# MilchRatchet/Luminary

Measured on AMD Instinct MI355X. Metric: Mrays/s at 1920x1080, 8 bounces, higher is better.
Workload: dtype f32

## Files before the change

include/lum_core.h:

```cpp
#ifndef LUM_CORE_H
#define LUM_CORE_H

#include <stdint.h>

#ifdef __cplusplus
extern "C" {
#endif

typedef struct LumContext LumContext;

typedef struct LumDeviceSceneView {
  uint32_t num_meshes;
  uint32_t num_instances;
  uint32_t num_materials;
  uint32_t num_lights;
  const uint32_t* mesh_tri_offset;
  const float* vertices;
  const uint32_t* tri_tex;
  const uint32_t* instance_mesh_ids;
  const float* instance_transforms;
  const uint16_t* materials;
  const uint8_t* light_tree_root;
  const uint8_t* light_tree_nodes;
  const uint32_t* light_tri_handles;
// ... 204 lines not shown
int lumc_frame_assemble(LumContext* ctx, uint32_t frame_pixels, int root, void* stream, float** d_frame_out);
int lumc_frame_assemble_all(LumContext** ctxs, int n, uint32_t frame_pixels, int root, float** d_frame_root);
int lumc_frame_gather(LumContext* ctx, uint32_t width, uint32_t height, int root, void* stream, float** d_frame_out);
int lumc_frame_gather_all(LumContext** ctxs, int n, uint32_t width, uint32_t height, int root, float** d_frame_root);
int lumc_frame_download(LumContext* ctx, uint32_t frame_pixels, float* first_moment, float* second_moment);
uint32_t lumc_frame_plane_stride(const LumContext* ctx);
int lumc_use_assembled_frame(LumContext* ctx, int on);
int lumc_accumulators_from_frame(LumContext* dst, LumContext* src);
int lumc_comm_count(const LumContext* ctx);
int lumc_device_name(int ordinal, char* out, size_t size);

int lumc_set_ray_sorting(LumContext* ctx, int mode);
int lumc_get_ray_sorting(const LumContext* ctx);

enum { LUMC_FLAVOUR_EXACT = 0, LUMC_FLAVOUR_FAST = 1 };
int lumc_set_flavour(LumContext* ctx, int flavour);
int lumc_get_flavour(const LumContext* ctx);
int lumc_set_ambient_reuse(LumContext* ctx, int mode);
int lumc_get_ambient_reuse(const LumContext* ctx);
int lumc_set_single_level(LumContext* ctx, int mode);
int lumc_get_single_level(const LumContext* ctx);
int lumc_set_plain_form(LumContext* ctx, int mode);
int lumc_get_plain_form(const LumContext* ctx);
int lumc_set_fused_resolve(LumContext* ctx, int on);
int lumc_set_sobol_table(LumContext* ctx, int on);
double lumc_bvh_build_seconds(const LumContext* ctx);
int lumc_bvh_meshes_by_builder(const LumContext* ctx, uint32_t out[2]);
int lumc_bvh_stats(LumContext* ctx, uint64_t out[4]);
uint32_t lumc_scene_view_sizeof(void);
int lumc_host_bvh_probe(const float* boxes, uint32_t count, uint32_t max_leaf, uint64_t out[6], double inner_area[3]);
uint32_t lumc_leaf_max_triangles(void);
typedef struct LumMeshRefitStats {
  uint64_t refits, rebuilds;
  uint32_t last_refits, last_rebuilds;
  double max_cost_growth;
  double seconds;
  double seconds_upload, seconds_refit, seconds_rebuild, seconds_assemble;
  double seconds_hash, seconds_download, seconds_lights;
} LumMeshRefitStats;
int lumc_set_mesh_refit(LumContext* ctx, uint32_t mode, float max_cost_growth);
int lumc_mesh_refit_stats(const LumContext* ctx, LumMeshRefitStats* out);
int lumc_bvh_refit_probe(const float* built_boxes, const float* refit_boxes, uint32_t count, uint32_t refit_count, int builder, int on_gpu, uint64_t sizes[3],
                         void* built_nodes, void* refit_nodes, void* host_refit_nodes, uint32_t* prims, double cost[3], uint64_t* valid);
int lumc_scene_tree_probe(const LumDeviceSceneView* scene, uint64_t sizes[4], void* nodes, void* tris, void* leaves, void* rows, uint32_t* mesh_root, float bounds[6]);
typedef struct LumInstanceUpdateStats {
  uint64_t device_updates, fallbacks, relayouts;
// ... 98 lines not shown
```

luminary_amd/core.py:

```python
import ctypes as C

import numpy as np

from . import DeviceSceneView, _lib

DIRTY_CONSTANTS, DIRTY_MATERIALS, DIRTY_INSTANCES, DIRTY_LIGHTS, DIRTY_MESHES, DIRTY_TEXTURES, DIRTY_PARTICLES, DIRTY_ALL = 1, 2, 4, 8, 16, 32, 64, 127
DIRTY_MESH_POSITIONS = 128
DIRTY_INSTANCE_TRANSFORMS = 256
DIRTY_MESH_SKIN = 512
DIRTY_LIGHT_POSITIONS = 1024
DIRTY_MESH_SHUTTER = 2048
BVH_BUILDERS = {"sah": 0, "lbvh": 1, "ploc": 2, "sah_gpu": 3}
CNT_TRACE, CNT_SHADOW, CNT_LIGHT_BVH, CNT_VERTICES, CNT_NODES, CNT_TRIS, CNT_NODES_SHADOW, CNT_TRIS_SHADOW, CNT_NODES_LIGHT, CNT_TRIS_LIGHT, CNT_NODES_LDS, CNT_NODES_LDS_SHADOW, CNT_AMBIENT_DEFERRED, CNT_AMBIENT_FALLBACK = range(14)
CNT_COUNT = 16
KERNELS = ("generate", "trace", "shade", "shadow", "accumulate", "light_query", "resolve", "output", "sky", "sort", "volume")


class CoreError(RuntimeError):
    pass


class OutputParams(C.Structure):
    _fields_ = [("src_width", C.c_uint32), ("src_height", C.c_uint32), ("dst_width", C.c_uint32), ("dst_height", C.c_uint32),
                ("inv_sample_count", C.c_float), ("exposure", C.c_float), ("tonemap", C.c_uint32), ("filter", C.c_uint32), ("dithering", C.c_uint32),
# ... 375 lines not shown

    @property
    def ambient_reuse(self):
        fn = self._lib.lumc_get_ambient_reuse
        fn.restype = C.c_int
        return bool(fn(self._ctx))

    def set_single_level(self, mode):
        self._call("lumc_set_single_level", C.c_int(mode))

    def get_single_level(self):
        fn = self._lib.lumc_get_single_level
        fn.restype = C.c_int
        return int(fn(self._ctx))

    def set_plain_form(self, mode):
        self._call("lumc_set_plain_form", C.c_int(mode))

    def get_plain_form(self):
        fn = self._lib.lumc_get_plain_form
        fn.restype = C.c_int
        return int(fn(self._ctx))

    def set_physical_camera(self, camera):
        self._call("lumc_set_physical_camera", C.byref(camera) if camera is not None else C.c_void_p(0))

    def camera_rays(self, pixels, first_sample, samples):
        px = np.ascontiguousarray(pixels, dtype=np.uint32)
        n = px.size * samples
        o = np.zeros((n, 3), dtype=np.float32)
        d = np.zeros((n, 3), dtype=np.float32)
        w = np.zeros(n, dtype=np.float32)
        self._call("lumc_camera_rays", px.ctypes.data_as(C.c_void_p), C.c_uint32(px.size), C.c_uint32(first_sample), C.c_uint32(samples),
                   o.ctypes.data_as(C.c_void_p), d.ctypes.data_as(C.c_void_p), w.ctypes.data_as(C.c_void_p))
        return o, d, w

    def pixel_query(self, x, y, sample_id=0):
        out = (C.c_uint32 * 6)()
        self._call("lumc_pixel_query", C.c_uint32(x), C.c_uint32(y), C.c_uint32(sample_id), out)
        a = np.array(list(out), dtype=np.uint32)
        return int(a[0]), int(a[1]), float(a[2:3].view(np.float32)[0]), a[3:6].view(np.float32).copy()

    def set_flavour(self, name):
        self._call("lumc_set_flavour", C.c_int({"exact": 0, "fast": 1}[name]))

    def _call(self, name, *args):
# ... 89 lines not shown
    def accumulators(self):
        fm = np.zeros(3 * self.num_pixels, dtype=np.float32)
        sm = np.zeros(self.num_pixels, dtype=np.float32)
        self._call("lumc_download_accumulators", fm.ctypes.data_as(C.c_void_p), sm.ctypes.data_as(C.c_void_p))
        return fm.reshape(3, -1), sm

    def counters(self):
        out = (C.c_uint64 * CNT_COUNT)()
        self._call("lumc_counters", out)
        return [int(x) for x in out]

    def query_counters(self):
        c = self.counters()
        c[CNT_SHADOW] += c[CNT_AMBIENT_DEFERRED] - c[CNT_AMBIENT_FALLBACK]
        return c

    def reset_counters(self):
        self._call("lumc_reset_counters")

    def set_profiling(self, on):
        self._call("lumc_set_profiling", C.c_int(1 if on else 0))

    def kernel_times(self):
        ms = (C.c_double * len(KERNELS))()
        n = (C.c_uint32 * len(KERNELS))()
        self._call("lumc_kernel_times", ms, n)
        return {k: (float(ms[i]), int(n[i])) for i, k in enumerate(KERNELS)}

    def adaptive_begin(self, max_rate, avg_rate, update_interval, exposure=0.0, tone=None):
        p = AdaptiveParams()
        p.max_sampling_rate, p.avg_sampling_rate, p.update_interval, p.exposure = max_rate, avg_rate, update_interval, exposure
        if tone is not None:
            p.tone = tone
        self._call("lumc_adaptive_begin", C.byref(p))

    def adaptive_render(self, executions, stream=0):
        self._call("lumc_adaptive_render", C.c_uint32(executions), C.c_void_p(stream))

    def adaptive_info(self):
        info = AdaptiveInfo()
        self._call("lumc_adaptive_info", C.byref(info))
        return {"stage_id": int(info.stage_id), "executions": [int(x) for x in info.executions], "num_blocks": int(info.num_blocks),
                "blocks": (int(info.blocks_x), int(info.blocks_y)), "tasks_per_execution": int(info.tasks_per_execution),
                "variance_total": float(info.variance_total), "build_pending": bool(info.build_pending)}

    @staticmethod
    def adaptive_info_of(ctx):
# ... 296 lines not shown
```

luminary_amd/csrc/device/wavefront_table.h:

```cpp
#pragma once

#include <hip/hip_runtime.h>

#include "dev_scene.h"

namespace lum {

inline bool single_level_scene(const DeviceScene& sc) { return sc.tlas_num_nodes == 1u && sc.tlas_num_leaves == 2u; }

inline bool plain_scene(const DeviceScene& sc) {
  return (sc.traits & kTraitsPlain) == kTraitsPlain && sc.num_lights <= (uint32_t) LUM_LDS_LIGHTS && !sc.ocean_active &&
         (sc.sky_mode == kSkyConstantColor || sc.sky_mode == kSkyHdri);
}

struct WavefrontKernels {
  const char* flavour;
  uint32_t trace_block;
  int (*set_ray_kernel_lds)(size_t bytes);
  int (*init_sampler_seeds)();
  void (*sobol_table)(hipStream_t s, uint2* table, uint32_t first_sample, uint32_t count, uint32_t stride, uint32_t dims);
  void (*generate)(uint32_t grid, hipStream_t s, const DeviceScene& sc, const PassParams& pp, const PathQueue& q, float4* results, uint32_t* count, const DeviceLens& lens,
                   int cam);
  void (*generate_adaptive)(uint32_t grid, hipStream_t s, const DeviceScene& sc, const AdaptiveView& a, const AdaptivePass& pass, const PathQueue& q, float4* results,
                            uint32_t* count, const DeviceLens& lens, int cam);
// ... 35 lines not shown
  void (*trace_rays)(uint32_t grid, size_t lds, hipStream_t s, const DeviceScene& sc, uint32_t n, const float* origins, const float* dirs, const uint32_t* ignore, uint32_t* out,
                     uint32_t* cursor, uint64_t* counters, uint32_t lds_nodes, bool single_level);
  void (*camera_rays)(uint32_t grid, hipStream_t s, const DeviceScene& sc, const DeviceLens& lens, int cam, const uint32_t* pixels, uint32_t n, uint32_t first_sample,
                      uint32_t samples, float* origin, float* dir, float* weight);
  void (*guide)(uint32_t grid, hipStream_t s, const DeviceScene& sc, const PathQueue& in, const uint32_t* ctrl, float* planes, uint32_t n);
  void (*guide_normalise)(uint32_t grid, hipStream_t s, float* planes, uint32_t n, uint32_t samples);
  void (*denoise_prepare)(uint32_t grid, hipStream_t s, const AdaptiveView& a, const DenoiseArgs& p, const float* fm, const float* sm, const float* image, const float* guides,
                          float4* rec_a, uint4* rec_b);
  void (*denoise_atrous)(hipStream_t s, const DenoiseArgs& p, const float4* a_in, const uint4* rec_b, float4* a_out, bool lds);
  void (*denoise_finish)(uint32_t grid, hipStream_t s, const DenoiseArgs& p, const float4* rec_a, const float* guides, float* image);
  void (*light_query_probe)(hipStream_t s, const DeviceScene& sc, uint32_t n, const float* origins, const float* dirs, const uint32_t* self, const float* randoms, uint32_t* out_ids,
                            uint32_t* out_num_hits);
};
struct WavefrontProbes {
  void (*light_sample_probe)(hipStream_t s, const DeviceScene& sc, uint32_t n_vertices, uint32_t samples, uint32_t first_sample, uint32_t form, const uint32_t* vertices,
                             uint32_t* out);
};
constexpr uint32_t kLightSampleProbeVertexWords = 20, kLightSampleProbeWords = 154;

const WavefrontKernels* wavefront_kernels_exact();
const WavefrontKernels* wavefront_kernels_fast();
const WavefrontProbes* wavefront_probes_exact();
const WavefrontProbes* wavefront_probes_fast();

}
```

luminary_amd/csrc/device/wavefront_table_impl.h:

```cpp
#pragma once

#include "dev_adaptive.h"
#include "dev_denoise.h"
#include "wavefront_table.h"

LUM_NS_BEGIN
namespace table {

typedef void (*TraceKernel)(DeviceScene, PathQueue, const uint32_t*, uint32_t*, uint64_t*, uint32_t);
typedef void (*ShadowKernel)(DeviceScene, ShadowQueue, const uint32_t*, uint32_t*, uint64_t*, uint32_t);
typedef void (*TraceRaysKernel)(DeviceScene, uint32_t, const float*, const float*, const uint32_t*, uint32_t*, uint32_t*, uint64_t*, uint32_t);
static TraceKernel trace_kernel(bool single) { return single ? k_trace<true> : static_cast<TraceKernel>(k_trace); }
static ShadowKernel shadow_kernel(bool single) { return single ? k_shadow_rays<true> : static_cast<ShadowKernel>(k_shadow_rays); }
static TraceRaysKernel trace_rays_kernel(bool single) { return single ? k_trace_rays<true> : static_cast<TraceRaysKernel>(k_trace_rays); }

static int set_ray_kernel_lds(size_t bytes) {
  hipError_t e = hipSuccess;
  for (int single = 0; single < 2 && e == hipSuccess; single++) {
    e = hipFuncSetAttribute((const void*) trace_kernel(single != 0), hipFuncAttributeMaxDynamicSharedMemorySize, (int) bytes);
    if (e == hipSuccess) e = hipFuncSetAttribute((const void*) shadow_kernel(single != 0), hipFuncAttributeMaxDynamicSharedMemorySize, (int) bytes);
    if (e == hipSuccess) e = hipFuncSetAttribute((const void*) trace_rays_kernel(single != 0), hipFuncAttributeMaxDynamicSharedMemorySize, (int) bytes);
  }
  if (e == hipSuccess) e = hipFuncSetAttribute((const void*) k_trace_particles, hipFuncAttributeMaxDynamicSharedMemorySize, (int) bytes);
  return (int) e;
}
static int init_sampler_seeds() { return upload_sampler_seeds(); }
static void sobol_table(hipStream_t s, uint2* table, uint32_t first_sample, uint32_t count, uint32_t stride, uint32_t dims) {
  hipLaunchKernelGGL(k_sobol_table, dim3((dims * stride + 255u) / 256u), dim3(256), 0, s, table, first_sample, count, stride, dims);
}
static void generate(uint32_t grid, hipStream_t s, const DeviceScene& sc, const PassParams& pp, const PathQueue& q, float4* results, uint32_t* count, const DeviceLens& lens,
                     int cam) {
  auto* k = cam == kCamPhysical ? k_generate<kCamPhysical> : cam == kCamPhysicalReflections ? k_generate<kCamPhysicalReflections> : k_generate<kCamThinLens>;
  hipLaunchKernelGGL(k, dim3(grid), dim3(kBlock), 0, s, sc, pp, q, results, count, lens);
}
static void generate_adaptive(uint32_t grid, hipStream_t s, const DeviceScene& sc, const AdaptiveView& a, const AdaptivePass& pass, const PathQueue& q, float4* results,
                              uint32_t* count, const DeviceLens& lens, int cam) {
  auto* k = cam == kCamPhysical ? k_generate_adaptive<kCamPhysical> : cam == kCamPhysicalReflections ? k_generate_adaptive<kCamPhysicalReflections>
                                                                                                     : k_generate_adaptive<kCamThinLens>;
  hipLaunchKernelGGL(k, dim3(grid), dim3(kBlock), 0, s, sc, a, pass, q, results, count, lens);
}
static void camera_rays(uint32_t grid, hipStream_t s, const DeviceScene& sc, const DeviceLens& lens, int cam, const uint32_t* pixels, uint32_t n, uint32_t first_sample,
                        uint32_t samples, float* origin, float* dir, float* weight) {
  auto* k = cam == kCamPhysical ? k_camera_rays<kCamPhysical> : cam == kCamPhysicalReflections ? k_camera_rays<kCamPhysicalReflections> : k_camera_rays<kCamThinLens>;
  hipLaunchKernelGGL(k, dim3(grid), dim3(kBlock), 0, s, sc, lens, pixels, n, first_sample, samples, origin, dir, weight);
}
static void trace(uint32_t grid, size_t lds, hipStream_t s, const DeviceScene& sc, const PathQueue& q, const uint32_t* order, uint32_t* ctrl, uint64_t* counters,
// ... 158 lines not shown
extern "C" int lumc_debug_vis_stats_fast(uint64_t out[8], int reset) {
  if (hipMemcpyFromSymbol(out, HIP_SYMBOL(g_vis_stat), sizeof(uint64_t) * 8) != hipSuccess) return 1;
  if (reset) { const uint64_t zero[8] = {0}; if (hipMemcpyToSymbol(HIP_SYMBOL(g_vis_stat), zero, sizeof(zero)) != hipSuccess) return 1; }
  return 0;
}
extern "C" int lumc_debug_shade_times_fast(uint64_t out[16], int reset) {
  if (hipMemcpyFromSymbol(out, HIP_SYMBOL(g_shade_time), sizeof(uint64_t) * 16) != hipSuccess) return 1;
  if (reset) { const uint64_t zero[16] = {0}; if (hipMemcpyToSymbol(HIP_SYMBOL(g_shade_time), zero, sizeof(zero)) != hipSuccess) return 1; }
  return 0;
}
#else
extern "C" int lumc_debug_phase_stats(uint64_t out[16], int reset) {
  if (hipMemcpyFromSymbol(out, HIP_SYMBOL(g_phase), sizeof(uint64_t) * 16) != hipSuccess) return 1;
  if (reset) { const uint64_t zero[16] = {0}; if (hipMemcpyToSymbol(HIP_SYMBOL(g_phase), zero, sizeof(zero)) != hipSuccess) return 1; }
  return 0;
}
#endif
#endif

namespace lum {
#if LUM_FAST
const WavefrontKernels* wavefront_kernels_fast() { return &fast::table::kTable; }
const WavefrontProbes* wavefront_probes_fast() { return &fast::table::kProbes; }
#else
const WavefrontKernels* wavefront_kernels_exact() { return &exact::table::kTable; }
const WavefrontProbes* wavefront_probes_exact() { return &exact::table::kProbes; }
#endif
}
```

luminary_amd/csrc/host/context.h:

```cpp
#pragma once

#include <hip/hip_runtime.h>

#include <cstdio>
#include <map>
#include <memory>
#include <string>
#include <vector>

#include "../../../include/lum_core.h"
#include "../device/dev_scene.h"
#include "../device/wavefront_table.h"
#include "bvh_build.h"
#include "bvh_refit.h"
#include "device_buffer.h"
#include "instance_update.h"
#include "light_refit.h"
#include "mesh_deform.h"
#include "mesh_shutter.h"
#include "scene_arrays.h"
#include "work_layout.h"

using namespace lum;

// ... 40 lines not shown
  DeviceBuffer<uint32_t> d_skin_flags;
  LumMeshSkinStats skin_stats{};
  LumMeshMorphStats morph_stats{};
  std::map<uint32_t, MeshShutter> mesh_shutter;
  DeviceBuffer<uint32_t> d_shutter_flags;
  LumShutterStats shutter_stats{};
  LightRefit light_refit;
  Bvh4 light_bvh;
  float light_refit_max_cost_growth = 0.0f;
  bool light_refit_needs_rebuild = false;
  bool lights_refitted = false;
  LumLightRefitStats light_refit_stats{};
  std::vector<uint32_t> sky_lut_key;
  DeviceBuffer<float> d_bridge_lut;
  std::vector<float> bridge_lut_host;
  DeviceBuffer<float4> d_sky_lut[2];
  DeviceScene scene{};
  bool has_scene = false;
  uint64_t bvh_stats[4] = {0, 0, 0, 0};
  int ambient_reuse = -1;
  int single_level = -1;
  int plain_form = -1;
  bool first_leaf_identity = false;
  uint32_t shade_grid_rounds = 2;
  int fused_resolve = 1;
  struct Fused : FusedBuffers {
    DeviceBuffer<char> block;
    bool records_stale = false;
    uint32_t refused_capacity = 0;
  } fused;
  DeviceBuffer<uint2> d_sobol;
  int sobol_table = 1;
  int fused_ended = 1;
  int fused_ended_default = 1;
  int bvh_builder = 3;
  double bvh_build_seconds = 0.0;
  uint32_t bvh_meshes_by_builder[2] = {0, 0};
  uint32_t lds_nodes = 0;
  uint32_t trace_blocks = 256;
  DeviceBuffer<uint16_t> d_luts[4];
  DeviceBuffer<uint32_t> d_pixels;
  uint32_t num_pixels = 0;
  uint64_t pixels_hash = 0;
  DeviceBuffer<float> d_first_moment, d_second_moment;
  struct Work : WorkBuffers { DeviceBuffer<char> block; } work;
  uint32_t particle_lds_nodes = 0;
// ... 62 lines not shown
};

#define HIP_TRY(ctx, expr)                                                                                          \
  do {                                                                                                              \
    const hipError_t e__ = (expr);                                                                                  \
    if (e__ != hipSuccess) {                                                                                        \
      (ctx)->error = std::string(#expr) + " failed: " + hipGetErrorString(e__);                                     \
      return 1;                                                                                                     \
    }                                                                                                               \
  } while (0)

#pragma GCC visibility push(hidden)

constexpr uint32_t kLaunchBlock = 256;
inline uint32_t grid_for(uint32_t n) {
  const uint32_t blocks = (n + kLaunchBlock - 1) / kLaunchBlock;
  return blocks < 1 ? 1 : (blocks > 2048 ? 2048 : blocks);
}

inline bool single_level_allowed(const LumContext* ctx) {
  return ctx->single_level != 0 && (ctx->wf != wavefront_kernels_fast() || ctx->first_leaf_identity);
}

inline uint32_t grid_persistent(const LumContext* ctx, uint32_t n) {
  const uint32_t tb = ctx->wf->trace_block;
  const uint32_t blocks = (n + tb - 1) / tb;
  return blocks < 1 ? 1 : (blocks > ctx->trace_blocks ? ctx->trace_blocks : blocks);
}

struct Launch {
  LumContext* ctx;
  hipStream_t stream;
  int kernel;
  size_t idx = (size_t) -1;
  Launch(LumContext* c, hipStream_t s, int k) : ctx(c), stream(s), kernel(k) {
    if (!ctx->profiling) return;
    LumContext::Stamp st;
    st.kernel = k;
    if (hipEventCreate(&st.a) != hipSuccess || hipEventCreate(&st.b) != hipSuccess) return;
    (void) hipEventRecord(st.a, stream);
    ctx->stamps.push_back(st);
    idx = ctx->stamps.size() - 1;
  }
  ~Launch() {
    if (idx != (size_t) -1) (void) hipEventRecord(ctx->stamps[idx].b, stream);
    if (ctx->sync_debug) {
// ... 17 lines not shown
```

luminary_amd/csrc/host/core.hip:

```cpp
#include <hip/hip_runtime.h>

#include <algorithm>
#include <cmath>
#include <cstdio>
#include <cstdlib>
#include <cstring>
#include <string>
#include <vector>

#include "../../../include/lum_core.h"
#include "../device/kernels_shared.h"
#include <hipcub/hipcub.hpp>
#include "context.h"
#include "tiles.h"

static_assert(kLaunchBlock == (uint32_t) kBlock, "grid_for (context.h) counts the kernels' workgroups");

namespace {

void free_work(LumContext* ctx) {
  ctx->work = LumContext::Work{};
  ctx->fused = LumContext::Fused{};
  free_sort(ctx);
  ctx->d_sobol.reset();
// ... 50 lines not shown

inline uint32_t shade_grid(const LumContext* ctx, uint32_t n) {
  const uint32_t blocks = (n + kBlock - 1) / kBlock;
  const uint32_t resident = ctx->trace_blocks * 3u;
  const uint32_t rounds = ctx->shade_grid_rounds;
  const uint32_t cap = resident * (rounds ? rounds : 1u);
  return blocks < 1 ? 1 : std::min(blocks, cap);
}

int resolve_stamps(LumContext* ctx) {
  for (auto& st : ctx->stamps) {
    float ms = 0.0f;
    if (hipEventSynchronize(st.b) == hipSuccess && hipEventElapsedTime(&ms, st.a, st.b) == hipSuccess) {
      ctx->kernel_ms[st.kernel] += ms;
      ctx->kernel_launches[st.kernel]++;
    }
    (void) hipEventDestroy(st.a);
    (void) hipEventDestroy(st.b);
  }
  ctx->stamps.clear();
  return 0;
}

}

extern "C" {

int lumc_context_create(int device_ordinal, LumContext** out) {
  if (!out) return 1;
  *out = nullptr;
  LumContext* ctx = new LumContext();
  ctx->device = device_ordinal;
  if (const char* b = getenv("LUM_BVH_BUILDER")) ctx->bvh_builder = (std::strcmp(b, "lbvh") == 0) ? 1 : (std::strcmp(b, "ploc") == 0) ? 2 : (std::strcmp(b, "sah") == 0 || std::strcmp(b, "host") == 0) ? 0 : 3;
  if (const char* e = getenv("LUM_SORT")) ctx->sort.mode = atoi(e);
  if (const char* e = getenv("LUM_SYNC_DEBUG")) ctx->sync_debug = atoi(e) != 0;
  if (const char* e = getenv("LUM_SORT_KEY")) ctx->sort.key = atoi(e);
  if (const char* e = getenv("LUM_AMBIENT_REUSE")) ctx->ambient_reuse = atoi(e) != 0 ? 1 : 0;
  if (const char* e = getenv("LUM_SINGLE_LEVEL")) ctx->single_level = atoi(e) != 0 ? 1 : 0;
  if (const char* e = getenv("LUM_PLAIN_FORM")) ctx->plain_form = atoi(e) != 0 ? 1 : 0;
  if (const char* e = getenv("LUM_FUSED_RESOLVE")) ctx->fused_resolve = atoi(e) != 0 ? 1 : 0;
  if (const char* e = getenv("LUM_SHADE_GRID")) ctx->shade_grid_rounds = (uint32_t) atoi(e);
  if (const char* e = getenv("LUM_SOBOL_TABLE_RT")) ctx->sobol_table = atoi(e) != 0 ? 1 : 0;
  if (const char* e = getenv("LUM_FUSED_ENDED")) ctx->fused_ended = ctx->fused_ended_default = atoi(e) != 0 ? 1 : 0;
  if (const char* e = getenv("LUM_DENOISE_LDS")) ctx->denoise_lds = atoi(e) != 0 ? 1 : 0;
  if (const char* f = getenv("LUM_FLAVOUR")) ctx->wf = (std::strcmp(f, "exact") == 0) ? wavefront_kernels_exact() : wavefront_kernels_fast();
  *out = ctx;
  int count = 0;
  HIP_TRY(ctx, hipGetDeviceCount(&count));
  if (device_ordinal < 0 || device_ordinal >= count) { ctx->error = "no such HIP device"; return 1; }
  HIP_TRY(ctx, hipSetDevice(device_ordinal));
  HIP_TRY(ctx, (hipError_t) wavefront_kernels_exact()->init_sampler_seeds());
  HIP_TRY(ctx, (hipError_t) wavefront_kernels_fast()->init_sampler_seeds());
  HIP_TRY(ctx, (hipError_t) exact::upload_sampler_seeds());
  HIP_TRY(ctx, (hipError_t) scene_device_init());
  HIP_TRY(ctx, ctx->d_ctrl.resize(kCtlStride * kCtrlRows));
  HIP_TRY(ctx, hipMemset(ctx->d_ctrl.get(), 0, sizeof(uint32_t) * kCtlStride * kCtrlRows));
  HIP_TRY(ctx, ctx->d_counters.resize(LUMC_CNT_COUNT));
  HIP_TRY(ctx, hipMemset(ctx->d_counters.get(), 0, sizeof(uint64_t) * LUMC_CNT_COUNT));
  return 0;
}

void lumc_context_destroy(LumContext* ctx) {
  if (!ctx) return;
  (void) hipSetDevice(ctx->device);
  (void) hipDeviceSynchronize();
  resolve_stamps(ctx);
  free_exchange(ctx);
  delete ctx;
}

const char* lumc_last_error(const LumContext* ctx) { return ctx ? ctx->error.c_str() : "null context"; }
uint32_t lumc_scene_view_sizeof(void) { return (uint32_t) sizeof(LumDeviceSceneView); }

uint64_t pixel_list_hash(const uint32_t* pixels, uint32_t n) {
  uint64_t h = 1469598103934665603ull;
  for (uint32_t i = 0; i < n; i++) { h ^= pixels ? pixels[i] : i; h *= 1099511628211ull; }
  return h;
}

int lumc_set_pixels(LumContext* ctx, const uint32_t* pixels, uint32_t num_pixels) {
  if (!ctx || !ctx->has_scene) { if (ctx) ctx->error = "lumc_set_pixels: no scene"; return 1; }
  HIP_TRY(ctx, hipSetDevice(ctx->device));
  if (!pixels) num_pixels = ctx->scene.width * ctx->scene.height;
  ctx->adaptive = LumContext::Adaptive();
  ctx->d_pixels.reset(); ctx->d_first_moment.reset(); ctx->d_second_moment.reset();
  ctx->num_pixels = num_pixels;
  ctx->pixels_hash = pixel_list_hash(pixels, num_pixels);
  if (num_pixels == 0) return 0;
  HIP_TRY(ctx, ctx->d_pixels.assign(pixels, num_pixels));
// ... 47 lines not shown
  if (sc.particles_active) trace_particles(ctx, stream, ctx->work.queue[0], ctx->d_ctrl.get(), N);
  if (sc.ocean_active) {
    Launch l(ctx, stream, LUMC_KERNEL_TRACE);
    wf.trace_ocean(grid_for(N), stream, sc, ctx->work.queue[0], (const uint32_t*) ctx->d_ctrl.get());
  }
}

static void debug_pass(LumContext* ctx, hipStream_t stream, const DeviceScene& sc, uint32_t N) {
  const WavefrontKernels& wf = *ctx->wf;
  first_hits(ctx, stream, sc, N);
  if (render_volumes(sc)) {
    Launch l(ctx, stream, LUMC_KERNEL_VOLUME);
    wf.volume_events(grid_for(N), stream, sc, ctx->work.queue[0], ctx->work.volume, ctx->work.results, ctx->d_ctrl.get(), 0u);
  }
  if (sc.sky_aerial_perspective && sc.sky_mode != kSkyConstantColor) {
    Launch l(ctx, stream, LUMC_KERNEL_SKY);
    wf.sky_inscattering(grid_for(N), stream, sc, ctx->work.queue[0], ctx->work.results, (const uint32_t*) ctx->d_ctrl.get(), 0u);
  }
  Launch l(ctx, stream, LUMC_KERNEL_SHADE);
  wf.shade_debug(grid_for(N), stream, sc, ctx->work.queue[0], ctx->work.results, (const uint32_t*) ctx->d_ctrl.get());
}

enum ResolveScheme { kResolvePlain, kResolveReuse, kResolveFused };

struct DepthBuffers {
  PathQueue& cur;
  PathQueue& next;
  PathQueue& prev;
  NeeQueue& nee;
  NeeQueue& nee_before;
  uint32_t* ctrl;
  const FusedResolve* fused_records;
  uint32_t* ended;
  uint32_t depth, depth_const;
  bool last;
};

static DepthBuffers depth_buffers(LumContext* ctx, ResolveScheme scheme, uint32_t depth, uint32_t max_depth) {
  const bool fused = scheme == kResolveFused;
  const int cur = fused ? (int) (depth % 3u) : (int) (depth & 1u);
  const int next_q = fused ? (cur + 1) % 3 : (cur ^ 1), prev_q = fused ? (cur + 2) % 3 : (cur ^ 1);
  const bool second_set = fused && (depth & 1u);
  const uint32_t depth_const = (depth == max_depth && depth > 0) ? depth - 1 : depth;
  return DepthBuffers{ctx->work.queue[cur], ctx->work.queue[next_q], ctx->work.queue[prev_q], second_set ? ctx->fused.nee : ctx->work.nee, second_set ? ctx->work.nee : ctx->fused.nee,
                      ctx->d_ctrl.get() + kCtlStride * depth, fused ? ctx->fused.records + depth % 6u : nullptr, fused ? ctx->fused.ended[depth & 1u] : nullptr, depth, depth_const,
                      depth == max_depth};
}

static int closest_hits(LumContext* ctx, hipStream_t stream, const DeviceScene& sc, ResolveScheme scheme, const DepthBuffers& d, uint32_t N) {
  const WavefrontKernels& wf = *ctx->wf;
  const uint32_t* order = nullptr;
  if (ctx->sort.mode >= 1 && d.depth >= 1 && sort_closest_rays(ctx, stream, d.cur, d.ctrl, N, &order)) return 1;
  {
    Launch l(ctx, stream, LUMC_KERNEL_TRACE);
    wf.trace(grid_persistent(ctx, N), ray_kernel_lds(ctx), stream, sc, d.cur, order, d.ctrl, ctx->d_counters.get(), ctx->lds_nodes, single_level_allowed(ctx));
  }
  if (scheme == kResolveReuse && d.depth > 0) {
    uint32_t* prev = d.ctrl - kCtlStride;
    {
      Launch l(ctx, stream, LUMC_KERNEL_RESOLVE);
      wf.resolve_reuse(grid_for(N), stream, sc, d.prev, d.cur, d.nee, ctx->work.shadow, ctx->work.results, prev, ctx->d_counters.get());
    }
    {
      Launch l(ctx, stream, LUMC_KERNEL_SHADOW);
      wf.shadow_rays(ctx->trace_blocks, ray_kernel_lds(ctx), stream, sc, ctx->work.shadow, nullptr, prev + kCtlVolumeShift, ctx->d_counters.get(), ctx->lds_nodes, single_level_allowed(ctx));
    }
    Launch l(ctx, stream, LUMC_KERNEL_RESOLVE);
    wf.resolve_listed(std::min<uint32_t>(grid_for(N), 1024u), stream, sc, d.prev, d.nee, ctx->work.shadow, ctx->work.results, (const uint32_t*) prev);
  }
  return 0;
}

static void media_passes(LumContext* ctx, hipStream_t stream, const DeviceScene& sc, const DepthBuffers& d, uint32_t N) {
  const WavefrontKernels& wf = *ctx->wf;
  if (sc.particles_active) trace_particles(ctx, stream, d.cur, d.ctrl, N);
  if (sc.ocean_active) {
    Launch l(ctx, stream, LUMC_KERNEL_TRACE);
    wf.trace_ocean(grid_for(N), stream, sc, d.cur, (const uint32_t*) d.ctrl);
  }
// ... 37 lines not shown
      wf.shadow_rays(ctx->trace_blocks, ray_kernel_lds(ctx), stream, sc, ctx->fused.fallback, nullptr, d.ctrl + kCtlVolumeShift, ctx->d_counters.get(), ctx->lds_nodes, single_level_allowed(ctx));
    }
    Launch l(ctx, stream, LUMC_KERNEL_RESOLVE);
    wf.resolve_listed(std::min<uint32_t>(grid_for(N), 1024u), stream, sc, d.prev, d.nee_before, ctx->fused.fallback, ctx->work.results, (const uint32_t*) d.ctrl);
  }
}

static void feature_shading(LumContext* ctx, hipStream_t stream, const DeviceScene& sc, const DepthBuffers& d, uint32_t N) {
  const WavefrontKernels& wf = *ctx->wf;
  if (sc.particles_active) {
    Launch l(ctx, stream, LUMC_KERNEL_SHADE);
    wf.particle_shade(grid_for(N), stream, sc, d.cur, d.next, d.nee, ctx->work.shadow, d.ctrl, d.depth_const);
  }
  if (sc.ocean_active) {
    Launch l(ctx, stream, LUMC_KERNEL_SHADE);
    wf.ocean_shade(grid_for(N), stream, sc, d.cur, d.next, d.nee, ctx->work.shadow, d.ctrl, d.depth_const);
  }
  if (sc.sky_mode == kSkyDefault) {
    Launch l(ctx, stream, LUMC_KERNEL_SKY);
    wf.sky(grid_for(N), stream, sc, d.cur, ctx->work.shadow, ctx->work.results, (const uint32_t*) d.ctrl, d.depth_const);
  }
}

static int visibility_and_resolve(LumContext* ctx, hipStream_t stream, const DeviceScene& sc, ResolveScheme scheme, const DepthBuffers& d, uint32_t N) {
  const WavefrontKernels& wf = *ctx->wf;
  {
    Launch l(ctx, stream, LUMC_KERNEL_LIGHT_QUERY);
    wf.light_query(std::min<uint32_t>(grid_for(N), ctx->trace_blocks * 4u), stream, sc, d.cur, d.nee, ctx->work.shadow, d.ctrl, d.depth_const, ctx->d_counters.get());
  }
  const uint32_t* shadow_order = nullptr;
  if (ctx->sort.mode == 2) {
    shadow_order = sort_rays(ctx, stream, ctx->work.shadow.origin_dist, ctx->work.shadow.dir_out, d.ctrl + kCtlShadowItems,
                             (sc.ocean_active ? kSurfaceShadowKindsWater : 4u) * (ctx->work.shadow.capacity < N ? ctx->work.shadow.capacity : N));
    if (!shadow_order) { ctx->error = "ray sorting failed"; return 1; }
  }
  {
    Launch l(ctx, stream, LUMC_KERNEL_SHADOW);
    wf.shadow_rays(grid_persistent(ctx, N), ray_kernel_lds(ctx), stream, sc, ctx->work.shadow, shadow_order, d.ctrl, ctx->d_counters.get(), ctx->lds_nodes, single_level_allowed(ctx));
  }
  if (d.last || scheme == kResolvePlain) {
    Launch l(ctx, stream, LUMC_KERNEL_RESOLVE);
    wf.resolve(grid_for(N), stream, sc, d.cur, d.nee, ctx->work.shadow, ctx->work.results, (const uint32_t*) d.ctrl);
  }
  else if (scheme == kResolveFused) {
    if (!ctx->fused_ended) {
      Launch l(ctx, stream, LUMC_KERNEL_RESOLVE);
      wf.resolve_ended(std::min<uint32_t>(grid_for(N), 4096u), stream, sc, d.cur, d.nee, ctx->work.shadow, ctx->work.results, (const uint32_t*) d.ctrl, d.ended);
    }
  }
  return 0;
}

static void volume_bounce(LumContext* ctx, hipStream_t stream, const DeviceScene& sc, const DepthBuffers& d, uint32_t N) {
  if (render_volumes(sc) && !d.last) {
    Launch l(ctx, stream, LUMC_KERNEL_VOLUME);
    ctx->wf->volume_bounce(grid_for(N), stream, sc, d.cur, d.next, ctx->work.volume, d.ctrl, d.depth_const);
  }
}

static int wavefront_depths(LumContext* ctx, hipStream_t stream, uint32_t N, uint32_t first_sample = 0, uint32_t sample_count = 0) {
  DeviceScene sc = ctx->scene;
  const uint32_t max_depth = sc.max_ray_depth;
  prepare_sobol_table(ctx, stream, sc, first_sample, sample_count);
  if (sc.shading_mode != 0u) { debug_pass(ctx, stream, sc, N); return 0; }
  ResolveScheme scheme = ambient_reuse_active(ctx) ? kResolveReuse : kResolvePlain;
  if (scheme == kResolveReuse && ctx->wf->fused_resolve && ctx->fused_resolve != 0 && ctx->wf == wavefront_kernels_fast() && max_depth > 0) {
    if (ensure_fused(ctx, stream) == 0) scheme = kResolveFused;
    else {
      (void) hipGetLastError();
      ctx->error.clear();
    }
  }
  for (uint32_t depth = 0; depth <= max_depth; depth++) {
    const DepthBuffers d = depth_buffers(ctx, scheme, depth, max_depth);
    if (closest_hits(ctx, stream, sc, scheme, d, N)) return 1;
    media_passes(ctx, stream, sc, d, N);
    shade_depth(ctx, stream, sc, scheme, d, N);
    feature_shading(ctx, stream, sc, d, N);
    if (visibility_and_resolve(ctx, stream, sc, scheme, d, N)) return 1;
    volume_bounce(ctx, stream, sc, d, N);
  }
  return 0;
}

int lumc_render(LumContext* ctx, uint32_t first_sample, uint32_t num_samples, uint32_t samples_per_pass, float* d_fm, float* d_sm, void* stream_) {
  if (!ctx || !ctx->has_scene) { if (ctx) ctx->error = "lumc_render: no scene"; return 1; }
  if (ctx->num_pixels == 0) return 0;
  hipStream_t stream = (hipStream_t) stream_;
  HIP_TRY(ctx, hipSetDevice(ctx->device));
  if (!d_fm) { d_fm = ctx->d_first_moment.get(); d_sm = ctx->d_second_moment.get(); }
  if (samples_per_pass == 0) samples_per_pass = 1;
  if (first_sample >= kMaxGlobalSamples) return 0;
  if (first_sample + (uint64_t) num_samples > kMaxGlobalSamples) num_samples = kMaxGlobalSamples - first_sample;
  const uint32_t P = ctx->num_pixels;
  const uint64_t want = (uint64_t) P * samples_per_pass;
  if (want > 0x7FFFFFFFull) { ctx->error = "pass too large"; return 1; }
  if (ensure_work(ctx, (uint32_t) want)) return 1;
  const DeviceScene& sc = ctx->scene;
  const uint32_t max_depth = sc.max_ray_depth;

  for (uint32_t done = 0; done < num_samples; done += samples_per_pass) {
// ... 857 lines not shown
  return 0;
}
int lumc_set_ambient_reuse(LumContext* ctx, int mode) {
  if (!ctx || mode < -1 || mode > 1) { if (ctx) ctx->error = "lumc_set_ambient_reuse: -1 (by flavour), 0 (off) or 1 (on)"; return 1; }
  ctx->ambient_reuse = mode;
  return 0;
}
int lumc_get_ambient_reuse(const LumContext* ctx) { return (ctx && ambient_reuse_active(ctx)) ? 1 : 0; }

int lumc_set_single_level(LumContext* ctx, int mode) {
  if (!ctx || mode < -1 || mode > 1) { if (ctx) ctx->error = "lumc_set_single_level: -1 (auto), 0 (never) or 1 (when the scene is eligible)"; return 1; }
  ctx->single_level = mode;
  return 0;
}
int lumc_get_single_level(const LumContext* ctx) { return (ctx && ctx->has_scene && single_level_allowed(ctx) && single_level_scene(ctx->scene)) ? 1 : 0; }

int lumc_set_plain_form(LumContext* ctx, int mode) {
  if (!ctx || mode < -1 || mode > 1) { if (ctx) ctx->error = "lumc_set_plain_form: -1 (auto), 0 (never) or 1 (when the scene is eligible)"; return 1; }
  ctx->plain_form = mode;
  return 0;
}

int lumc_get_plain_form(const LumContext* ctx) { return (ctx && ctx->has_scene && ctx->plain_form != 0 && plain_scene(ctx->scene)) ? 1 : 0; }
int lumc_get_flavour(const LumContext* ctx) { return (ctx && ctx->wf == wavefront_kernels_exact()) ? LUMC_FLAVOUR_EXACT : LUMC_FLAVOUR_FAST; }

unsigned int lumc_lds_stack_bytes(void) { return LUM_LDS_STACK_BYTES; }

}
```

Before: 4137.

## Overlap light queries with next-depth trace on a side stream

```diff
diff --git a/include/lum_core.h b/include/lum_core.h
--- a/include/lum_core.h
+++ b/include/lum_core.h
@@ -250,6 +250,9 @@
 int lumc_get_single_level(const LumContext* ctx);
 int lumc_set_plain_form(LumContext* ctx, int mode);
 int lumc_get_plain_form(const LumContext* ctx);
+int lumc_set_overlap_light_query(LumContext* ctx, int mode);
+int lumc_get_overlap_light_query(const LumContext* ctx);
+int lumc_overlap_registers_fit(uint32_t ray_kernel_regs, uint32_t light_query_regs);
 int lumc_set_fused_resolve(LumContext* ctx, int on);
 int lumc_set_sobol_table(LumContext* ctx, int on);
 double lumc_bvh_build_seconds(const LumContext* ctx);
diff --git a/luminary_amd/core.py b/luminary_amd/core.py
--- a/luminary_amd/core.py
+++ b/luminary_amd/core.py
@@ -421,6 +421,20 @@
         fn.restype = C.c_int
         return int(fn(self._ctx))
 
+    def set_overlap_light_query(self, mode):
+        self._call("lumc_set_overlap_light_query", C.c_int(mode))
+
+    def get_overlap_light_query(self):
+        fn = self._lib.lumc_get_overlap_light_query
+        fn.restype = C.c_int
+        return int(fn(self._ctx))
+
+    @staticmethod
+    def overlap_registers_fit(ray_kernel_regs, light_query_regs):
+        fn = _lib().lumc_overlap_registers_fit
+        fn.restype = C.c_int
+        return bool(fn(C.c_uint32(ray_kernel_regs), C.c_uint32(light_query_regs)))
+
     def set_physical_camera(self, camera):
         self._call("lumc_set_physical_camera", C.byref(camera) if camera is not None else C.c_void_p(0))
 
@@ -556,7 +570,7 @@
         self._call("lumc_set_profiling", C.c_int(1 if on else 0))
 
     def kernel_times(self):
-        ms = (C.c_double * len(KERNELS))()
+        ms =(C.c_double * len(KERNELS))()
         n = (C.c_uint32 * len(KERNELS))()
         self._call("lumc_kernel_times", ms, n)
         return {k: (float(ms[i]), int(n[i])) for i, k in enumerate(KERNELS)}
diff --git a/luminary_amd/csrc/device/wavefront_table.h b/luminary_amd/csrc/device/wavefront_table.h
--- a/luminary_amd/csrc/device/wavefront_table.h
+++ b/luminary_amd/csrc/device/wavefront_table.h
@@ -81,5 +81,7 @@
 const WavefrontKernels* wavefront_kernels_fast();
 const WavefrontProbes* wavefront_probes_exact();
 const WavefrontProbes* wavefront_probes_fast();
+int ray_kernel_registers_exact(bool single_level, uint32_t* trace_regs, uint32_t* light_query_regs);
+int ray_kernel_registers_fast(bool single_level, uint32_t* trace_regs, uint32_t* light_query_regs);
 
 }
diff --git a/luminary_amd/csrc/device/wavefront_table_impl.h b/luminary_amd/csrc/device/wavefront_table_impl.h
--- a/luminary_amd/csrc/device/wavefront_table_impl.h
+++ b/luminary_amd/csrc/device/wavefront_table_impl.h
@@ -22,6 +22,15 @@
     if (e == hipSuccess) e = hipFuncSetAttribute((const void*) trace_rays_kernel(single != 0), hipFuncAttributeMaxDynamicSharedMemorySize, (int) bytes);
   }
   if (e == hipSuccess) e = hipFuncSetAttribute((const void*) k_trace_particles, hipFuncAttributeMaxDynamicSharedMemorySize, (int) bytes);
+  return (int) e;
+}
+static int ray_kernel_registers(bool single_level, uint32_t* trace_regs, uint32_t* light_query_regs) {
+  hipFuncAttributes a{};
+  hipError_t e = hipFuncGetAttributes(&a, (const void*) trace_kernel(single_level));
+  if (e != hipSuccess) return (int) e;
+  *trace_regs = (uint32_t) a.numRegs;
+  e = hipFuncGetAttributes(&a, (const void*) k_light_query);
+  if (e == hipSuccess) *light_query_regs = (uint32_t) a.numRegs;
   return (int) e;
 }
 static int init_sampler_seeds() { return upload_sampler_seeds(); }
@@ -226,7 +235,9 @@
 #if LUM_FAST
 const WavefrontKernels* wavefront_kernels_fast() { return &fast::table::kTable; }
 const WavefrontProbes* wavefront_probes_fast() { return &fast::table::kProbes; }
+int ray_kernel_registers_fast(bool single_level, uint32_t* trace_regs, uint32_t* light_query_regs) { return fast::table::ray_kernel_registers(single_level, trace_regs, light_query_regs); }
 #else
+int ray_kernel_registers_exact(bool single_level, uint32_t* trace_regs, uint32_t* light_query_regs) { return exact::table::ray_kernel_registers(single_level, trace_regs, light_query_regs); }
 const WavefrontKernels* wavefront_kernels_exact() { return &exact::table::kTable; }
 const WavefrontProbes* wavefront_probes_exact() { return &exact::table::kProbes; }
 #endif
diff --git a/luminary_amd/csrc/host/context.h b/luminary_amd/csrc/host/context.h
--- a/luminary_amd/csrc/host/context.h
+++ b/luminary_amd/csrc/host/context.h
@@ -86,6 +86,10 @@
   int single_level = -1;
   int plain_form = -1;
   bool first_leaf_identity = false;
+  int overlap_lq = -1;
+  hipStream_t side_stream = nullptr;
+  std::vector<hipEvent_t> overlap_events;
+  bool overlap_fits[2][2] = {{false, false}, {false, false}};
   uint32_t shade_grid_rounds = 2;
   int fused_resolve = 1;
   struct Fused : FusedBuffers {
@@ -194,6 +198,11 @@
   return ctx->single_level != 0 && (ctx->wf != wavefront_kernels_fast() || ctx->first_leaf_identity);
 }
 
+inline bool overlap_registers_fit(uint32_t ray_kernel_regs, uint32_t light_query_regs) {
+  const uint32_t ray = (ray_kernel_regs + 7u) & ~7u, lq = (light_query_regs + 7u) & ~7u;
+  return ray_kernel_regs > 0 && light_query_regs > 0 && 4u * ray + lq <= 512u;
+}
+
 inline uint32_t grid_persistent(const LumContext* ctx, uint32_t n) {
   const uint32_t tb = ctx->wf->trace_block;
   const uint32_t blocks = (n + tb - 1) / tb;
diff --git a/luminary_amd/csrc/host/core.hip b/luminary_amd/csrc/host/core.hip
--- a/luminary_amd/csrc/host/core.hip
+++ b/luminary_amd/csrc/host/core.hip
@@ -96,6 +96,28 @@
   return 0;
 }
 
+void prepare_overlap(LumContext* ctx) {
+  int least = 0, greatest = 0;
+  if (hipDeviceGetStreamPriorityRange(&least, &greatest) != hipSuccess) least = 0;
+  if (hipStreamCreateWithPriority(&ctx->side_stream, hipStreamNonBlocking, least) != hipSuccess) ctx->side_stream = nullptr;
+  for (int fast = 0; fast < 2; fast++)
+    for (int single = 0; single < 2; single++) {
+      uint32_t trace_regs = 0, light_query_regs = 0;
+      const int e = fast ? ray_kernel_registers_fast(single != 0, &trace_regs, &light_query_regs) : ray_kernel_registers_exact(single != 0, &trace_regs, &light_query_regs);
+      ctx->overlap_fits[fast][single] = e == 0 && overlap_registers_fit(trace_regs, light_query_regs);
+    }
+  (void) hipGetLastError();
+}
+
+int ensure_overlap_events(LumContext* ctx, uint32_t depths) {
+  while (ctx->overlap_events.size() < 2u * (size_t) depths) {
+    hipEvent_t e;
+    HIP_TRY(ctx, hipEventCreateWithFlags(&e, hipEventDisableTiming));
+    ctx->overlap_events.push_back(e);
+  }
+  return 0;
+}
+
 }
 
 extern "C" {
@@ -112,6 +134,7 @@
   if (const char* e = getenv("LUM_AMBIENT_REUSE")) ctx->ambient_reuse = atoi(e) != 0 ? 1 : 0;
   if (const char* e = getenv("LUM_SINGLE_LEVEL")) ctx->single_level = atoi(e) != 0 ? 1 : 0;
   if (const char* e = getenv("LUM_PLAIN_FORM")) ctx->plain_form = atoi(e) != 0 ? 1 : 0;
+  if (const char* e = getenv("LUM_OVERLAP_LQ")) ctx->overlap_lq = atoi(e) != 0 ? 1 : 0;
   if (const char* e = getenv("LUM_FUSED_RESOLVE")) ctx->fused_resolve = atoi(e) != 0 ? 1 : 0;
   if (const char* e = getenv("LUM_SHADE_GRID")) ctx->shade_grid_rounds = (uint32_t) atoi(e);
   if (const char* e = getenv("LUM_SOBOL_TABLE_RT")) ctx->sobol_table = atoi(e) != 0 ? 1 : 0;
@@ -131,6 +154,7 @@
   HIP_TRY(ctx, hipMemset(ctx->d_ctrl.get(), 0, sizeof(uint32_t) * kCtlStride * kCtrlRows));
   HIP_TRY(ctx, ctx->d_counters.resize(LUMC_CNT_COUNT));
   HIP_TRY(ctx, hipMemset(ctx->d_counters.get(), 0, sizeof(uint64_t) * LUMC_CNT_COUNT));
+  prepare_overlap(ctx);
   return 0;
 }
 
@@ -139,6 +163,8 @@
   (void) hipSetDevice(ctx->device);
   (void) hipDeviceSynchronize();
   resolve_stamps(ctx);
+  for (hipEvent_t e : ctx->overlap_events) (void) hipEventDestroy(e);
+  if (ctx->side_stream) (void) hipStreamDestroy(ctx->side_stream);
   free_exchange(ctx);
   delete ctx;
 }
@@ -232,6 +258,20 @@
 }
 
 enum ResolveScheme { kResolvePlain, kResolveReuse, kResolveFused };
+
+static ResolveScheme wanted_scheme(const LumContext* ctx) {
+  if (!ambient_reuse_active(ctx)) return kResolvePlain;
+  return (ctx->wf->fused_resolve && ctx->fused_resolve != 0 && ctx->wf == wavefront_kernels_fast() && ctx->scene.max_ray_depth > 0) ? kResolveFused : kResolveReuse;
+}
+
+constexpr bool kOverlapAuto = true;
+static bool overlap_allowed(const LumContext* ctx, ResolveScheme scheme) {
+  const DeviceScene& sc = ctx->scene;
+  const bool wanted = ctx->overlap_lq < 0 ? kOverlapAuto : ctx->overlap_lq != 0;
+  if (!wanted || !ctx->has_scene || !ctx->side_stream || scheme == kResolveReuse || ctx->sort.mode != 0 || sc.shading_mode != 0u || sc.max_ray_depth == 0u) return false;
+  if (sc.fog_active || sc.ocean_active || sc.particles_active || sc.cloud_active || sc.sky_aerial_perspective) return false;
+  return ctx->overlap_fits[ctx->wf == wavefront_kernels_fast() ? 1 : 0][(single_level_allowed(ctx) && single_level_scene(sc)) ? 1 : 0];
+}
 
 struct DepthBuffers {
   PathQueue& cur;
@@ -257,14 +297,16 @@
                       depth == max_depth};
 }
 
+static void trace_depth(LumContext* ctx, hipStream_t stream, const DeviceScene& sc, const DepthBuffers& d, const uint32_t* order, uint32_t N) {
+  Launch l(ctx, stream, LUMC_KERNEL_TRACE);
+  ctx->wf->trace(grid_persistent(ctx, N), ray_kernel_lds(ctx), stream, sc, d.cur, order, d.ctrl, ctx->d_counters.get(), ctx->lds_nodes, single_level_allowed(ctx));
+}
+
 static int closest_hits(LumContext* ctx, hipStream_t stream, const DeviceScene& sc, ResolveScheme scheme, const DepthBuffers& d, uint32_t N) {
   const WavefrontKernels& wf = *ctx->wf;
   const uint32_t* order = nullptr;
   if (ctx->sort.mode >= 1 && d.depth >= 1 && sort_closest_rays(ctx, stream, d.cur, d.ctrl, N, &order)) return 1;
-  {
-    Launch l(ctx, stream, LUMC_KERNEL_TRACE);
-    wf.trace(grid_persistent(ctx, N), ray_kernel_lds(ctx), stream, sc, d.cur, order, d.ctrl, ctx->d_counters.get(), ctx->lds_nodes, single_level_allowed(ctx));
-  }
+  trace_depth(ctx, stream, sc, d, order, N);
   if (scheme == kResolveReuse && d.depth > 0) {
     uint32_t* prev = d.ctrl - kCtlStride;
     {
@@ -348,12 +390,14 @@
   }
 }
 
+static void light_queries(LumContext* ctx, hipStream_t stream, const DeviceScene& sc, const DepthBuffers& d, uint32_t N, bool beside_trace) {
+  Launch l(ctx, stream, LUMC_KERNEL_LIGHT_QUERY);
+  const uint32_t per_cu = beside_trace ? 1u : 4u;
+  ctx->wf->light_query(std::min<uint32_t>(grid_for(N), ctx->trace_blocks * per_cu), stream, sc, d.cur, d.nee, ctx->work.shadow, d.ctrl, d.depth_const, ctx->d_counters.get());
+}
+
 static int visibility_and_resolve(LumContext* ctx, hipStream_t stream, const DeviceScene& sc, ResolveScheme scheme, const DepthBuffers& d, uint32_t N) {
   const WavefrontKernels& wf = *ctx->wf;
-  {
-    Launch l(ctx, stream, LUMC_KERNEL_LIGHT_QUERY);
-    wf.light_query(std::min<uint32_t>(grid_for(N), ctx->trace_blocks * 4u), stream, sc, d.cur, d.nee, ctx->work.shadow, d.ctrl, d.depth_const, ctx->d_counters.get());
-  }
   const uint32_t* shadow_order = nullptr;
   if (ctx->sort.mode == 2) {
     shadow_order = sort_rays(ctx, stream, ctx->work.shadow.origin_dist, ctx->work.shadow.dir_out, d.ctrl + kCtlShadowItems,
@@ -389,20 +433,35 @@
   const uint32_t max_depth = sc.max_ray_depth;
   prepare_sobol_table(ctx, stream, sc, first_sample, sample_count);
   if (sc.shading_mode != 0u) { debug_pass(ctx, stream, sc, N); return 0; }
-  ResolveScheme scheme = ambient_reuse_active(ctx) ? kResolveReuse : kResolvePlain;
-  if (scheme == kResolveReuse && ctx->wf->fused_resolve && ctx->fused_resolve != 0 && ctx->wf == wavefront_kernels_fast() && max_depth > 0) {
-    if (ensure_fused(ctx, stream) == 0) scheme = kResolveFused;
-    else {
-      (void) hipGetLastError();
-      ctx->error.clear();
-    }
-  }
+  ResolveScheme scheme = wanted_scheme(ctx);
+  if (scheme == kResolveFused && ensure_fused(ctx, stream) != 0) {
+    (void) hipGetLastError();
+    ctx->error.clear();
+    scheme = kResolveReuse;
+  }
+  const bool overlap = overlap_allowed(ctx, scheme) && ensure_overlap_events(ctx, max_depth) == 0;
+  hipStream_t side = ctx->side_stream;
+  bool traced = false;
   for (uint32_t depth = 0; depth <= max_depth; depth++) {
     const DepthBuffers d = depth_buffers(ctx, scheme, depth, max_depth);
-    if (closest_hits(ctx, stream, sc, scheme, d, N)) return 1;
+    if (!traced && closest_hits(ctx, stream, sc, scheme, d, N)) return 1;
+    traced = false;
     media_passes(ctx, stream, sc, d, N);
     shade_depth(ctx, stream, sc, scheme, d, N);
     feature_shading(ctx, stream, sc, d, N);
+    if (overlap && !d.last) {
+      hipEvent_t shaded = ctx->overlap_events[2u * depth], queried = ctx->overlap_events[2u * depth + 1u];
+      HIP_TRY(ctx, hipEventRecord(shaded, stream));
+      HIP_TRY(ctx, hipStreamWaitEvent(side, shaded, 0));
+      light_queries(ctx, side, sc, d, N, true);
+      const hipError_t recorded = hipEventRecord(queried, side);
+      if (recorded != hipSuccess) (void) hipStreamSynchronize(side);
+      HIP_TRY(ctx, recorded);
+      trace_depth(ctx, stream, sc, depth_buffers(ctx, scheme, depth + 1u, max_depth), nullptr, N);
+      traced = true;
+      HIP_TRY(ctx, hipStreamWaitEvent(stream, queried, 0));
+    }
+    else light_queries(ctx, stream, sc, d, N, false);
     if (visibility_and_resolve(ctx, stream, sc, scheme, d, N)) return 1;
     volume_bounce(ctx, stream, sc, d, N);
   }
@@ -1306,6 +1365,14 @@
 }
 
 int lumc_get_plain_form(const LumContext* ctx) { return (ctx && ctx->has_scene && ctx->plain_form != 0 && plain_scene(ctx->scene)) ? 1 : 0; }
+
+int lumc_set_overlap_light_query(LumContext* ctx, int mode) {
+  if (!ctx || mode < -1 || mode > 1) { if (ctx) ctx->error = "lumc_set_overlap_light_query: -1 (auto), 0 (never) or 1 (when the pass allows it)"; return 1; }
+  ctx->overlap_lq = mode;
+  return 0;
+}
+int lumc_get_overlap_light_query(const LumContext* ctx) { return (ctx && ctx->has_scene && overlap_allowed(ctx, wanted_scheme(ctx))) ? 1 : 0; }
+int lumc_overlap_registers_fit(uint32_t ray_kernel_regs, uint32_t light_query_regs) { return overlap_registers_fit(ray_kernel_regs, light_query_regs) ? 1 : 0; }
 int lumc_get_flavour(const LumContext* ctx) { return (ctx && ctx->wf == wavefront_kernels_exact()) ? LUMC_FLAVOUR_EXACT : LUMC_FLAVOUR_FAST; }
 
 unsigned int lumc_lds_stack_bytes(void) { return LUM_LDS_STACK_BYTES; }
```

New measurement: 4203 (median of 6 runs). 1.02x the previous value.
